# CloudEngineHub/MARL-LLM

Measured on AMD Instinct MI355X. Metric: agent-steps/sec, higher is better.
Workload: dtype f64 (state, every index / flag / reward decision) + f32 (obs, prior, action I/O, pre-filters); 1 GPU; assembly env, 64 agents x 4096 envs per GPU (64 x 4096 total), assembled state, prior-policy actions; agents=64, envs_per_gpu=4096, envs_total=4096, obs_dtype=f32, state_dtype=f64, seed=226, parallelism=env-sharded x1, no collective on the step path

## Files before the change

marl_llm_amd/csrc/swarm_env.hip:

```cpp

#include <hip/hip_runtime.h>

#include <cmath>
#include <cstdint>
#include <cstring>
#include <string>
#include <type_traits>
#include <utility>

#include "swarm_env.h"
#include "env_types.h"

using namespace swarm_internal;

#if !defined(SWARM_ENV_UNIT)
#define SWARM_UNIT_KERNELS 1
#define SWARM_UNIT_HOST 1
#elif SWARM_ENV_UNIT == 0
#define SWARM_UNIT_KERNELS 0
#define SWARM_UNIT_HOST 1
#else
#define SWARM_UNIT_KERNELS 1
#define SWARM_UNIT_HOST 0
#endif
// ... 725 lines not shown
                d2u = (act && up != 0) ? fmaf(dxu, dxu, dy2) : INFINITY;
                d2d = (act && dn != 0) ? fmaf(dxd, dxd, dy2) : INFINITY;
                c_dn = rs[b] + popc(dn) - 1;
            };
            for (int b = wr; b < nr_hi; b += WS) {
                float d2d, d2u; int c_dn;
                row_cands(b, d2d, d2u, c_dn);
                second32 = __builtin_amdgcn_fmed3f(best32, second32, d2d);
                bool lt = d2d < best32;
                best32 = lt ? d2d : best32; bc = lt ? c_dn : bc;
                second32 = __builtin_amdgcn_fmed3f(best32, second32, d2u);
                lt = d2u < best32;
                best32 = lt ? d2u : best32; bc = lt ? c_dn + 1 : bc;
            }
            const float lat_dlt = 1.2e-7f * fmaxf(fabsf(apf), fabsf(bpf)) + 2e-6f;
            const float tol = 6.0f * sqrtf(second32) * lat_dlt + 1e-9f;
            const bool unc_min = act && (wave_exact || (second32 < INFINITY && (second32 - best32) <= tol));
            if (__any(unc_min)) {
                if (unc_min) {
                    const float thr = wave_exact ? INFINITY : best32 + tol;
                    double bestd = INFINITY; int bcd = bc;
                    for (int b = wr; b < nr_hi; b += WS) {
                        float d2d, d2u; int c_dn;
                        row_cands(b, d2d, d2u, c_dn);
                        const bool td = d2d <= thr, tu = d2u <= thr && d2u < INFINITY;
                        if ((td && d2d < INFINITY) || tu) {
                            const double2 g0 = cell64((td && d2d < INFINITY) ? c_dn : 0), g1 = cell64(tu ? c_dn + 1 : 0);
                            const double e0x = g0.x - px, e0y = g0.y - py, e1x = g1.x - px, e1y = g1.y - py;
                            const double q0 = e0x * e0x + e0y * e0y, q1 = e1x * e1x + e1y * e1y;
                            if (td && d2d < INFINITY && q0 < bestd) { bestd = q0; bcd = c_dn; }
                            if (tu && q1 < bestd) { bestd = q1; bcd = c_dn + 1; }
                        }
                    }
                    bc = bcd;
                }
            }
        }
        };
        if (sx != SB || WPE == 1) { if (P.lat_n32) walk(0u); else walk((u64)0); }
    } else {
    for (int rep = 0, reps = REPS(3); rep < reps; ++rep) {
    FENCE();
    best32 = INFINITY; second32 = INFINITY; bc = 0;
    for (int w = 0; w < W; ++w) {
        if (!mine(w)) continue;
        unsigned word = 0, rword = 0;
        int mlo = 0, mhi = 0;
        int bl = 0; const float best_in = best32;
        unsigned orw = 0;
        const unsigned nlo = (unsigned)nearby1, nhi = (unsigned)(nearby1 >> 32);
        u64 unc = 0;
        const float4 *cq = reinterpret_cast<const float4 *>(cq_e + w * 64);
        static_for<16>([&](auto prc) {
            constexpr int pr = decltype(prc)::value;
            const float4 q = cq[pr];
            const f2v gx = {q.x, q.y}, gy = {q.z, q.w};
            const f2v rx = gx - pxx, ry = gy - pyy;
            const f2v d2v = __builtin_elementwise_fma(rx, rx, ry * ry);
            static_for<2>([&](auto hc) {
                constexpr int hh = decltype(hc)::value;
                constexpr int b = 2 * pr + hh;
                const float d2 = hh ? d2v.y : d2v.x;
                second32 = __builtin_amdgcn_fmed3f(best32, second32, d2);
                const bool lt = d2 < best32;
                best32 = lt ? d2 : best32;
                bl = lt ? b : bl;
                const u64 m_slo = __ballot(d2 < P.csen_lo), m_shi = __ballot(d2 < P.csen_hi);
                const u64 m_olo = __ballot(d2 < P.cocc_lo), m_ohi = __ballot(d2 < P.cocc_hi);
                rword = shl1_or_mask(rword, m_slo);
                if constexpr (NW == 1) {
                    const unsigned t = ((unsigned)m_olo & nlo) | ((unsigned)(m_olo >> 32) & nhi);
                    orw = shl1_or_mask(orw, __ballot(t != 0));
                } else {
                    mlo = writelane_c<b>((int)(unsigned)m_olo, mlo);
                    mhi = writelane_c<b>((int)(unsigned)(m_olo >> 32), mhi);
                }
                unc |= (m_slo ^ m_shi) | (m_olo ^ m_ohi);
            });
        });
        word = __brev(rword);
        unsigned oword = __brev(orw);
        if (best32 < best_in) bc = w * 32 + bl;
        u64 mym = ((u64)(unsigned)mhi << 32) | (unsigned)mlo;
        if (unc != 0 || wave_exact) {
            word = 0; oword = 0;
#pragma unroll 4
            for (int b = 0; b < 32; ++b) {
                const double2 g = cell64(w * 32 + b);
                const double rx = g.x - px, ry = g.y - py;
                const double d2 = rx * rx + ry * ry;
                if (d2 < P.c_sen) word |= 1u << b;
                const u64 m = __ballot(d2 < P.c_occ);
                if (lane == b) mym = m;
                if (NW == 1 && ((((unsigned)m & nlo) | ((unsigned)(m >> 32) & nhi)) != 0)) oword |= 1u << b;
            }
        }
        sbits[w * AG + at] = word;
        if constexpr (NW == 1) owords[w * AG + at] = oword;
        else if (lane < 32) cmask[(size_t)(w * 32 + lane) * NW + aw] = mym;
    }
    }
    {
        const float tol = P.min_tol_a * sqrtf(second32) + P.min_tol_b * second32 + 1e-9f;
        const bool unc_min = act && (wave_exact || (second32 < INFINITY && (second32 - best32) <= tol));
        if (__any(unc_min)) {
            const float thr = unc_min ? (wave_exact ? INFINITY : best32 + tol) : -1.0f;
            double bestd = INFINITY; int bcd = bc;
            for (int w = 0; w < W; ++w) {
                if (!mine(w)) continue;
                for (int b = 0; b < 32; ++b) {
                    const int cc = w * 32 + b;
                    const float rx = cq_e[(cc >> 1) * 4 + (cc & 1)] - pxf, ry = cq_e[(cc >> 1) * 4 + 2 + (cc & 1)] - pyf;
                    if (fmaf(rx, rx, ry * ry) <= thr || (wave_exact && unc_min)) {
                        const double2 g = cell64(w * 32 + b);
                        const double ex = g.x - px, ey = g.y - py;
                        const double d2 = ex * ex + ey * ey;
                        if (d2 < bestd) { bestd = d2; bcd = w * 32 + b; }
                    }
                }
            }
            if (unc_min) bc = bcd;
        }
    }
    }
    part_c[sx * AG + at] = (pc_t)bc;
    double *part_d = reinterpret_cast<double *>(smem + LO(partd));
    if constexpr (LAT) {
        if (sx != SB || WPE == 1) {
            const double2 g = cell64(bc);
            const double ex = g.x - px, ey = g.y - py;
            part_d[(WPE > 1 && sx > SB ? sx - 1 : sx) * AG + at] = ex * ex + ey * ey;
        }
    }
    STAMP(16);
    EXIT_AT(4);
    __syncthreads();
    STAMP(17);
    double best = INFINITY; bc = 0;
    for (int rep = 0, reps = REPS(12); rep < reps; ++rep) {
    FENCE();
    best = INFINITY; bc = 0;
#pragma unroll
    for (int s = 0; s < WPE; ++s) {
        if (LAT && WPE > 1 && s == SB) continue;
        const int c = part_c[s * AG + at];
        double d;
        if constexpr (LAT) d = part_d[(WPE > 1 && s > SB ? s - 1 : s) * AG + at];
        else { const double2 g = cell64(c); const double ex = g.x - px, ey = g.y - py; d = ex * ex + ey * ey; }
        if (d < best || (d == best && c < bc)) { best = d; bc = c; }
    }
    }
    const bool in_shape = act && best < P.c_in[es];
    if (sx == 0) {
        sncf[at] = bc | (in_shape ? (1 << 30) : 0);
        if (P.export_small && act) {
            P.near_cell[(size_t)e * n_a + i] = bc;
            P.in_flag[(size_t)e * n_a + i] = in_shape ? 1 : 0;
        }
    }
    STAMP(4);
    EXIT_AT(5);

    const int PPR = P.obs_dim >> 1;
    const int HP = 2 * (P.with_self + P.topo) + 2;
    const int envs_here = (P.n_env - blockIdx.x * EPB) < EPB ? (P.n_env - blockIdx.x * EPB) : EPB;
    const int rows = envs_here * n_a;
    OT2 *out = reinterpret_cast<OT2 *>(obs) + (size_t)blockIdx.x * EPB * n_a * PPR;

    auto prior_policy = [&]() {
    if (sx == SB && P.with_prior) {
        double qx = 0.0, qy = 0.0;
        double lx = 0.0, ly = 0.0;
        {
            const int ncf = sncf[at];
            double tx = px - px, ty = py - py;
            if (!(ncf >> 30)) { const double2 g = cell64(ncf & 0xFFFF); tx = g.x - px; ty = g.y - py; }
            const double dt_ = sqrt(tx * tx + ty * ty);
            if (dt_ > 0) { qx += P.pk_att * tx / dt_; qy += P.pk_att * ty / dt_; }
            lx = qx; ly = qy;
            double avx = 0.0, avy = 0.0; int cnt = 0;
#pragma unroll
            for (int k = 0; k < kTopoMax; ++k) {
                const int j = snei[at * kNeiStride + k];
                const bool used = j >= 0;
                const int tj = el * NPAD + (used ? j : 0);
                const double x = px - sp[tj], y = py - sp[AG + tj];
                const double d2n = x * x + y * y;
                if (used && d2n > 0 && d2n < P.c_avoid) {
                    const double d = sqrt(d2n);
                    const double ux = x / d, uy = y / d;
                    const double factor = P.pk_rep * (P.r_avoid / d - 1.0);
                    qx += factor * ux; qy += factor * uy;
                    if (P.llm) { const double fl = P.pk_llm * (P.r_avoid / d - 1.0); lx += fl * ux; ly += fl * uy; }
                }
                if (used) { avx += sp[2 * AG + tj]; avy += sp[3 * AG + tj]; ++cnt; }
            }
            if (cnt > 0) {
                avx /= cnt; avy /= cnt;
                const double sxv = P.pk_ali * (avx - sp[2 * AG + at]), syv = P.pk_ali * (avy - sp[3 * AG + at]);
                qx += sxv; qy += syv; lx += sxv; ly += syv;
            }
        }
        if (act) {
            OT2 o; o.x = to_out<OT>(clamp_ref(qx, -1.0, 1.0)); o.y = to_out<OT>(clamp_ref(qy, -1.0, 1.0));
            reinterpret_cast<OT2 *>(P.prior_next)[(size_t)e * n_a + i] = o;
            if (P.llm) { double2 u; u.x = clamp_ref(lx, -1.0, 1.0); u.y = clamp_ref(ly, -1.0, 1.0); P.act_next[(size_t)e * n_a + i] = u; }
        }
    }
    };

    auto head_blocks = [&](bool early) {
        for (int rep = 0, reps = REPS(7); rep < reps; ++rep) {
            FENCE();
            typedef OT OT4 __attribute__((ext_vector_type(4)));
            const int NB = P.with_self + P.topo + 1;
            const int total = rows * NB;
            const bool b_out = WPE > 1 && P.with_prior != 0;
            const int HT = b_out ? T - AG : T;
            const int ps = tid / AG, ps_b = (SB + WPE - (int)(blockIdx.x % WPE)) % WPE;
            const int htid = b_out ? (ps < ps_b ? ps : ps - 1) * AG + at : tid;
            const int n_it = early ? (total + 63) >> 6 : (total + HT - 1) / HT;
            for (int it_ = 0; it_ < n_it; ++it_) {
                int item;
                if (early) {
                    const int c8 = it_ & 7, owner = c8 < 5 ? 0 : 2;
                    const int k = owner == 0 ? 5 * (it_ >> 3) + c8 : 3 * (it_ >> 3) + c8 - 5;
                    if (sx != owner || (k % NW) != aw) continue;
                    item = it_ * 64 + lane;
                } else {
                    if (b_out && sx == SB) break;
                    item = htid + it_ * HT;
                }
                if (item < total) {
                    const int r = NB == 8 ? item >> 3 : item / NB, blk = item - r * NB;
                    const int elr = EPB > 1 ? r / n_a : 0;
                    const int tr = elr * NPAD + (r - elr * n_a);
                    const double ox = sp[tr], oy = sp[AG + tr], ou = sp[2 * AG + tr], ov = sp[3 * AG + tr];
                    const bool is_tgt = blk == NB - 1, is_nei = !is_tgt && !(P.with_self && blk == 0);
                    const int nslot = blk - P.with_self;
                    const int j = snei[tr * kNeiStride + (is_nei ? nslot : 0)];
                    const int ncf = sncf[tr];
                    const double2 g = P.cells_xy[(size_t)(blockIdx.x * EPB + elr) * P.ng_max + (ncf & 0xFFFF)];
                    const int tj = elr * NPAD + (j < 0 ? 0 : j);
                    const double nx = sp[tj], ny = sp[AG + tj], nu = sp[2 * AG + tj], nv = sp[3 * AG + tj];
                    const bool has = is_nei && j >= 0, out_t = is_tgt && !(ncf >> 30);
                    const bool zero_m = is_nei && !has;
                    double mx = has ? nx : (out_t ? g.x : ox), my = has ? ny : (out_t ? g.y : oy);
                    double mu = has ? nu : (out_t ? 0.0 : ou), mv = has ? nv : (out_t ? 0.0 : ov);
                    if (zero_m) { mx = 0.0; my = 0.0; mu = 0.0; mv = 0.0; }
                    const bool sub_own = has || is_tgt;
                    const double qx = sub_own ? ox : 0.0, qy = sub_own ? oy : 0.0, qu = sub_own ? ou : 0.0, qv = sub_own ? ov : 0.0;
                    double a = mx - qx, b = my - qy;
                    if (P.periodic && is_nei) wrap_rel(a, b, P.w_half, P.h_half);
                    OT2 *dst = out + (size_t)r * PPR + 2 * blk;
                    if ((PPR & 1) == 0) {
                        const OT4 o = {to_out<OT>(a), to_out<OT>(b), to_out<OT>(mu - qu), to_out<OT>(mv - qv)};
                        __builtin_nontemporal_store(o, reinterpret_cast<OT4 *>(dst));
                    } else {
                        OT2 o0, o1;
                        o0.x = to_out<OT>(a); o0.y = to_out<OT>(b); o1.x = to_out<OT>(mu - qu); o1.y = to_out<OT>(mv - qv);
                        store_nt(dst, o0); store_nt(dst + 1, o1);
                    }
                }
            }
        }
    };

    auto exact_uniform = [&](int La, int nL, int eL) -> bool {
        const double inv_dsen = 1.0 / P.d_sen;
        const double2 *gcl = P.cells_xy + (size_t)eL * P.ng_max;
        const double pxl = sp[La], pyl = sp[AG + La];
        const short *rowl = sidx + (size_t)La * P.g_stride;
        auto bcast = [](double v, int t) -> double {
            const u64 b = __builtin_bit_cast(u64, v);
            const unsigned lo = (unsigned)__builtin_amdgcn_readlane((int)(unsigned)b, t);
            const unsigned hi = (unsigned)__builtin_amdgcn_readlane((int)(unsigned)(b >> 32), t);
            return __builtin_bit_cast(double, ((u64)hi << 32) | lo);
        };
        double a0 = 0.0, a1 = 0.0, a2 = 0.0;
        for (int base = 0; base < nL; base += 64) {
            const int q = base + lane;
            double t0 = 0.0, t1 = 0.0, t2 = 0.0;
            if (q < nL) {
                const int cc = rowl[q];
                const double2 gq = gcl[cc];
                const double x = gq.x - pxl, y = gq.y - pyl;
                const double z = sqrt(x * x + y * y);
                const double psi = z < P.d_sen ? 0.5 * (1.0 + cospi01(z * inv_dsen)) : 0.0;
                t0 = psi * x; t1 = psi * y; t2 = psi;
            }
            const int m = nL - base < 64 ? nL - base : 64;
            for (int t = 0; t < m; ++t) { a0 += bcast(t0, t); a1 += bcast(t1, t); a2 += bcast(t2, t); }
        }
        if (a2 == 0) a2 = 1E-8;
        const double v0 = 1.0 * a0 / a2, v1 = 1.0 * a1 / a2;
        return sqrt(v0 * v0 + v1 * v1) < 0.05;
    };

    auto sensed_rows = [&](bool own, const unsigned char *pw) {
        for (int rep = 0, reps = REPS(8); rep < reps; ++rep) {
            FENCE();
            const int Gp = P.g_max;
            const int wv = __builtin_amdgcn_readfirstlane(tid >> 6), nwv = T >> 6;
            auto locate = [&](int k, int &tr, int &elr, int &r) -> bool {
                if (own) {
                    const int ta = (at & ~63) + pw[(64 - ACTW) + sx * AGW + k];
                    const int ii = NPAD < 64 ? (ta & 63) % NPAD : ta;
                    elr = NPAD < 64 ? (ta & 63) / NPAD : 0;
                    tr = ta; r = elr * n_a + ii;
                    return (blockIdx.x * EPB + elr) < P.n_env && ii < n_a;
                }
                r = k;
                const bool ok = r < rows;
                const int rq = ok ? r : rows - 1;
                elr = EPB > 1 ? rq / n_a : 0;
                tr = elr * NPAD + (rq - elr * n_a);
                return ok;
            };
            if (Gp == 80 && sizeof(OT) <= 4) {
                typedef OT OT4 __attribute__((ext_vector_type(4)));
                const int ngrp = own ? AGW / 8 : (rows + nwv * 8 - 1) / (nwv * 8);
                for (int g8 = 0; g8 < ngrp; ++g8) {
#pragma unroll
                    for (int ps = 0; ps < 5; ++ps) {
                        const int ch = ps * 64 + lane;
                        const int rl = (ch * 205) >> 13;
                        const int m = ch - rl * 40;
                        int tr, elr, r;
                        const bool ok = locate(own ? g8 * 8 + rl : (wv + g8 * nwv) * 8 + rl, tr, elr, r);
                        const double2 *gr = P.cells_xy + (size_t)(blockIdx.x * EPB + elr) * P.ng_max;
                        const double qx = sp[tr], qy = sp[AG + tr];
                        const int cc = *reinterpret_cast<const int *>(sidx + (size_t)tr * P.g_stride + 2 * m);
                        const int c0 = (int)(short)(cc & 0xFFFF), c1 = cc >> 16;
                        const double2 g0 = gr[c0 < 0 ? 0 : c0], g1 = gr[c1 < 0 ? 0 : c1];
                        const OT z = to_out<OT>(0.0);
                        const OT a0 = to_out<OT>(g0.x - qx), b0 = to_out<OT>(g0.y - qy);
                        const OT a1 = to_out<OT>(g1.x - qx), b1 = to_out<OT>(g1.y - qy);
                        OT4 o = {c0 >= 0 ? a0 : z, c0 >= 0 ? b0 : z, c1 >= 0 ? a1 : z, c1 >= 0 ? b1 : z};
                        if (ok) __builtin_nontemporal_store(o, reinterpret_cast<OT4 *>(out + (size_t)r * PPR + HP + 2 * m));
                    }
                }
            } else {
                const int nrow = own ? AGW : (rows - wv + nwv - 1) / nwv;
                for (int k = 0; k < nrow; ++k) {
                    int tr, elr, r;
                    const bool ok = locate(own ? k : wv + k * nwv, tr, elr, r);
                    const double2 *gr = P.cells_xy + (size_t)(blockIdx.x * EPB + elr) * P.ng_max;
                    const double qx = sp[tr], qy = sp[AG + tr];
                    const short *srw = sidx + (size_t)tr * P.g_stride;
                    for (int q = lane; q < Gp; q += 64) {
                        const int c = srw[q];
                        const double2 g = gr[c < 0 ? 0 : c];
                        OT2 o; o.x = c >= 0 ? to_out<OT>(g.x - qx) : to_out<OT>(0.0); o.y = c >= 0 ? to_out<OT>(g.y - qy) : to_out<OT>(0.0);
                        if (ok) store_nt(&out[(size_t)r * PPR + HP + q], o);
                    }
                }
            }
        }
    };

    const int G = P.g_max;
    int n_sel = 0;
    bool uniform = false, unsure = false;
    if constexpr (LAT) {
    const float4 hq = hdr[at];
    const int hb0 = __float_as_int(hq.z), hca0 = __float_as_int(hq.w);
    const LatEnv &L = P.lat[es];
    const u64 *rm = lrm + el * 64;
    const short *rs = lrs + el * 64;
    const bool flg = flag_get();
    for (int rep = 0, reps = REPS(4); rep < reps; ++rep) {
        FENCE();
        for (int t = sx; t < P.lat_nrs; t += WPE) {
            const int b = hb0 + t;
            const int bq = b < 0 ? 0 : (b > 63 ? 63 : b);
            const unsigned sel = srow[t * AG + at] & 0x1FFFFu;
            const u64 rowm = rm[bq];
            const int base = rs[bq] + __popcll(rowm & ((1ull << hca0) - 1ull));
            unsigned kept = sel;
            if (in_shape) {
                const unsigned cv = (unsigned)(covrow[el * 64 + bq] >> hca0);
                kept = sel & ~cv;
                if (flg) {
                    const unsigned relm = (unsigned)(rowm >> hca0);
                    unsigned it = sel & cv;
                    kept = sel;
                    while (it) {
                        const int c = __ffs(it) - 1; it &= it - 1;
                        const double2 g = cell64(base + __popc(relm & ((1u << c) - 1u)));
                        bool occ = false;
                        for (int q = 0; q < NW && !occ; ++q) {
                            u64 nbm = NW == 1 ? (nearby1 >> (NPAD < 64 ? el * NPAD : 0)) : snear[q * AG + at];
                            while (nbm && !occ) {
                                const int j = q * 64 + __ffsll((unsigned long long)nbm) - 1; nbm &= nbm - 1;
                                const double ex = g.x - spx[j], ey = g.y - spy[j];
                                occ = ex * ex + ey * ey < P.c_occ;
                            }
                        }
                        if (occ) kept &= ~(1u << c);
                    }
                }
            }
            if (rep == reps - 1) srow[t * AG + at] = kept | ((unsigned)base << 17);
            pcr[at * NRC + t] = (unsigned char)__popc(kept);
            if (P.export_idx) orow[t * AG + at] = sel & ~kept;
        }
    }
    {
        uint4 *fill = reinterpret_cast<uint4 *>(sidx);
        const int n16 = (AG * P.g_stride * 2) >> 4;
        for (int q = tid; q < n16; q += T) fill[q] = uint4{0xFFFFFFFFu, 0xFFFFFFFFu, 0xFFFFFFFFu, 0xFFFFFFFFu};
    }
    __syncthreads();
    STAMP(5);
    EXIT_AT(6);

    pc_t *prk = part_c;
    int n_kept;
    {
        const uint4 cq = reinterpret_cast<const uint4 *>(pcr)[at];
        n_kept = (int)__builtin_amdgcn_sad_u8(cq.x, 0u, __builtin_amdgcn_sad_u8(cq.y, 0u, __builtin_amdgcn_sad_u8(cq.z, 0u, __builtin_amdgcn_sad_u8(cq.w, 0u, 0u))));
        const int key = (lane < ACTW) ? n_kept * 64 + lane : lane - 64;
        int cnt = 0;
#pragma unroll
        for (int q = 0; q < 16; ++q) cnt += (__builtin_amdgcn_readlane(key, sx * 16 + q) < key) ? 1 : 0;
        prk[sx * AG + at] = (pc_t)cnt;
    }
    n_sel = n_kept > G ? G : n_kept;
    __syncthreads();
    STAMP(18);
    EXIT_AT(7);
    int ea;
    {
        int rank = 0;
#pragma unroll
        for (int s = 0; s < WPE; ++s) rank += prk[s * AG + at];
        unsigned char *pw = perm + (tid >> 6) * 64;
        pw[rank] = (unsigned char)lane;
        __builtin_amdgcn_fence(__ATOMIC_RELEASE, "wavefront");
        __builtin_amdgcn_wave_barrier();
        __builtin_amdgcn_fence(__ATOMIC_ACQUIRE, "wavefront");
        ea = (at & ~63) + pw[(64 - ACTW) + sx * AGW + lane / LPA];
    }
    { if (sx == 3) __builtin_amdgcn_s_setprio(3); else if (sx == 2) __builtin_amdgcn_s_setprio(2); else if (sx == SB) __builtin_amdgcn_s_setprio(1); }

    float qn0 = 0.0f, qn1 = 0.0f, qdn = 0.0f, qrl = 1.0f; int qnk = 0;
    for (int rep = 0, reps = REPS(11); rep < reps; ++rep) {
        FENCE();
        const int sub = lane & (LPA - 1);
        const float4 ha = hdr[ea];
        const float apr = ha.x, bpr = ha.y;
        const int ab0 = __float_as_int(ha.z), aca0 = __float_as_int(ha.w);
        const int ael = NPAD < 64 ? (ea & 63) / NPAD : 0;
        const LatEnv &La = P.lat[(blockIdx.x * EPB + ael) < P.n_env ? (blockIdx.x * EPB + ael) : P.n_env - 1];
        const float Rl = La.R;
        const float inv_r = __builtin_amdgcn_rcpf(Rl);
        const float apr_s = apr * inv_r;
        const u64 *rma = lrm + ael * 64;
        const uint4 cq = reinterpret_cast<const uint4 *>(pcr)[ea];
        const int s0 = (int)__builtin_amdgcn_sad_u8(cq.x, 0u, 0u), s1 = (int)__builtin_amdgcn_sad_u8(cq.y, 0u, 0u);
        const int s2 = (int)__builtin_amdgcn_sad_u8(cq.z, 0u, 0u), s3 = (int)__builtin_amdgcn_sad_u8(cq.w, 0u, 0u);
        const int nk = s0 + s1 + s2 + s3;
        const int per = (nk + LPA - 1) / LPA;
        const int k0 = sub * per < nk ? sub * per : nk;
        const int k1 = k0 + per < nk ? k0 + per : nk;
        int t, before;
        {
            const int c1 = s0, c2 = s0 + s1, c3 = c2 + s2;
            const int d = (k0 >= c1 ? 1 : 0) + (k0 >= c2 ? 1 : 0) + (k0 >= c3 ? 1 : 0);
            before = d == 0 ? 0 : (d == 1 ? c1 : (d == 2 ? c2 : c3));
            const unsigned wd = d == 0 ? cq.x : (d == 1 ? cq.y : (d == 2 ? cq.z : cq.w));
            const int e1 = before + (int)(wd & 255u), e2 = e1 + (int)((wd >> 8) & 255u), e3 = e2 + (int)((wd >> 16) & 255u);
            const int j = (k0 >= e1 ? 1 : 0) + (k0 >= e2 ? 1 : 0) + (k0 >= e3 ? 1 : 0);
            before = j == 0 ? before : (j == 1 ? e1 : (j == 2 ? e2 : e3));
            t = 4 * d + j;
        }
        const unsigned *srp = srow + t * AG + ea;
        const unsigned wd0 = *srp;
        unsigned kept = k0 < k1 ? (wd0 & 0x1FFFFu) : 0u;
        {
            int pb = 0, left = k0 - before;
#pragma unroll
            for (int sh = 16; sh >= 1; sh >>= 1) {
                const int c = __popc((kept >> pb) & ((1u << sh) - 1u));
                const bool go = left >= c;
                left -= go ? c : 0; pb += go ? sh : 0;
            }
            kept &= ~((1u << pb) - 1u);
        }
        int base = (int)(wd0 >> 17);
        const int bt0 = ab0 + t;
        const u64 *rmp = rma + (bt0 < 0 ? 0 : (bt0 > 63 ? 63 : bt0));
        unsigned relm = (unsigned)(*rmp >> aca0);
        float dbf = ((float)t - bpr) * inv_r, db2 = dbf * dbf;
        float n0 = 0.0f, n1 = 0.0f, dn = 0.0f;
        short *row = sidx + (size_t)ea * P.g_stride;
        const unsigned nm1 = (unsigned)(nk - 1);
        auto rank_of = [&](int q) -> int {
            if (P.cap_int) {
                const unsigned x = 2u * (unsigned)q * nm1 + (unsigned)(G - 1);
                const unsigned hq_ = __umulhi(x, P.cap_magic);
                return (int)((((x - hq_) >> 1) + hq_) >> P.cap_shift);
            }
            const double v = q * ((double)nm1 / (G - 1));
            return (int)(P.cap_even ? rint(v) : round(v));
        };
        auto walk_range = [&](auto capped) {
            constexpr bool CAP = decltype(capped)::value;
            int k = k0;
            int slot = k0, nxt = 0;
            if constexpr (CAP) {
                if (nk > G) {
                    if (P.cap_int) slot = k0 > 0 ? (int)((unsigned)((2 * k0 - 1) * (G - 1) + 2 * (int)nm1 - 1) / (2u * nm1)) : 0;
                    else { slot = 0; while (slot < G && rank_of(slot) < k0) ++slot; }
                    slot = slot < G ? slot : G;
                    nxt = slot < G ? rank_of(slot) : 0x7FFFFFFF;
                }
            }
            while (__any(k < k1)) {
                if (k < k1) {
                    if (kept == 0) {
                        srp += AG; ++rmp;
                        const unsigned wd = *srp;
                        kept = wd & 0x1FFFFu; base = (int)(wd >> 17);
                        relm = (unsigned)(*rmp >> aca0);
                        dbf += inv_r; db2 = dbf * dbf;
                    }
                    if (kept != 0) {
                        const int c = __ffs(kept) - 1;
                        kept &= kept - 1;
                        const int cell = base + __popc(relm & ((1u << c) - 1u));
                        bool take = true;
                        if constexpr (CAP) {
                            if (nk > G) {
                                take = k == nxt;
                                if (take) nxt = slot + 1 < G ? rank_of(slot + 1) : 0x7FFFFFFF;
                            }
                        }
                        if constexpr (CAP) { if (take) row[slot] = (short)cell; slot += take ? 1 : 0; }
                        else row[k] = (short)cell;
                        ++k;
                        const float da = fmaf((float)c, inv_r, -apr_s);
                        const float u = fmaf(da, da, db2);
                        float psi = psi5_u_f32(u);
                        if constexpr (CAP) psi = take ? psi : 0.0f;
                        n0 = fmaf(psi, da, n0); n1 = fmaf(psi, dbf, n1); dn += psi;
                    }
                }
            }
        };
        if (__any(nk > G)) walk_range(std::true_type{}); else walk_range(std::false_type{});
        auto quad_sum = [](float v) -> float {
            v += __int_as_float(__builtin_amdgcn_update_dpp(0, __float_as_int(v), 0xB1, 0xF, 0xF, true));
            v += __int_as_float(__builtin_amdgcn_update_dpp(0, __float_as_int(v), 0x4E, 0xF, 0xF, true));
            return v;
        };
        auto lanes_sum = [&](float v) -> float {
            v = quad_sum(v);
            if constexpr (LPA == 8) v += __int_as_float(__builtin_amdgcn_update_dpp(0, __float_as_int(v), 0x104, 0xF, 0xF, true));
            return v;
        };
        qn0 = lanes_sum(n0); qn1 = lanes_sum(n1); qdn = lanes_sum(dn); qnk = nk; qrl = Rl;
    }
    STAMP(19);
    EXIT_AT(9);
    __builtin_amdgcn_fence(__ATOMIC_RELEASE, "wavefront");
    __builtin_amdgcn_wave_barrier();
    __builtin_amdgcn_fence(__ATOMIC_ACQUIRE, "wavefront");
    {
        const int nsl = qnk > G ? G : qnk;
        const bool in_a = (sncf[ea] >> 30) != 0;
        const int ael = NPAD < 64 ? (ea & 63) / NPAD : 0, ai = NPAD < 64 ? (ea & 63) % NPAD : ea;
        const int ae = blockIdx.x * EPB + ael;
        const bool lead = (lane & (LPA - 1)) == 0 && ae < P.n_env && ai < n_a;
        const bool has = lead && in_a && nsl > 0;
        const float thr = P.rew_thr_k;
        const float idn = __builtin_amdgcn_rcpf(qdn);
        const float v0f = qn0 * idn, v1f = qn1 * idn;
        const float vf = sqrtf(fmaf(v0f, v0f, v1f * v1f));
        bool uni = has && vf < thr;
        const float inv_rl = __builtin_amdgcn_rcpf(qrl);
        const bool uns = has && (P.force_exact || !(qdn > 1e-6f) || !(fabsf(vf - thr) > (P.rew_ga_lat * (float)nsl * idn + P.rew_gb_lat) * inv_rl * 1.0001f));
        u64 um = __ballot(uns);
        while (um != 0) {
            const int L = __ffsll((unsigned long long)um) - 1;
            um &= um - 1;
            const bool res = exact_uniform(__builtin_amdgcn_readlane(ea, L), __builtin_amdgcn_readlane(nsl, L), __builtin_amdgcn_readlane(ae, L));
            if (lane == L) uni = res;
        }
        if (lead) {
            const size_t oi = (size_t)ae * n_a + ai;
            if (reward != nullptr) __builtin_nontemporal_store((in_a && !(snei[ea * kNeiStride + kTopoMax] != 0) && uni) ? 1.0f : 0.0f, &reward[oi]);
            if (done != nullptr) __builtin_nontemporal_store((uint8_t)0, &done[oi]);
        }
    }
    STAMP(6);
    EXIT_AT(10);
    prior_policy();
    if (obs != nullptr) {
        head_blocks(NW == 1);
        STAMP(9);
        EXIT_AT(11);
        sensed_rows(true, perm + (tid >> 6) * 64);
    }
    } else {
    {
        u64 nearby[NW];
#pragma unroll
        for (int q = 0; q < NW; ++q) nearby[q] = (NW > 1 && in_shape) ? snear[q * AG + at] : 0;
        for (int rep = 0, reps = REPS(4); rep < reps; ++rep)
        for (int w = 0; w < W; ++w) {
            if (!mine(w)) continue;
            FENCE();
            const unsigned word = sbits[w * AG + at];
            unsigned kw = word;
            if constexpr (NW == 1) {
                if (in_shape) kw = word & ~owords[w * AG + at];
                if (rep == reps - 1) sbits[w * AG + at] = kw;
            } else if (in_shape) {
                unsigned it = word;
                while (it) {
                    int bb[4]; bool occ[4];
#pragma unroll
                    for (int u = 0; u < 4; ++u) { bb[u] = it ? __ffs(it) - 1 : -1; it &= it - 1; }
#pragma unroll
                    for (int u = 0; u < 4; ++u) {
                        const int c = w * 32 + (bb[u] < 0 ? 0 : bb[u]);
                        occ[u] = false;
#pragma unroll
                        for (int q = 0; q < NW; ++q) occ[u] = occ[u] || ((cmask[(size_t)c * NW + q] & nearby[q]) != 0);
                    }
#pragma unroll
                    for (int u = 0; u < 4; ++u) if (bb[u] >= 0 && occ[u]) kw &= ~(1u << bb[u]);
                }
                if (rep == reps - 1) sbits[w * AG + at] = kw;
            }
            asm volatile("" :: "v"(kw));
            if (P.export_idx) obits[w * AG + at] = word & ~kw;
            pc[w * AG + at] = (unsigned char)__popc(kw);
        }
    }
    __syncthreads();
    STAMP(5);
    EXIT_AT(6);

    int n_kept = 0;
    for (int w = 0; w < W; ++w) n_kept += pc[w * AG + at];
    n_sel = n_kept > G ? G : n_kept;
    unsigned *rsel = reinterpret_cast<unsigned *>(smem + P.off_cmask);
    for (int w = sx; w <= W; w += WPE) rsel[w * AG + at] = 0;
    __syncthreads();
    const bool any_sub = __any(n_kept > G) != 0;
    int *sub_base = reinterpret_cast<int *>(smem + P.off_partc);
// ... 476 lines not shown
```

Baseline: 3.143 billion agent-steps/s.

## Software-pipeline the sensed-cell row gather with a four-deep load queue

For the own-agent path with full 64-agent padding, the 80-cell sensed-row emission is rewritten as a three-stage software pipeline. Index loads, the gathers of cell coordinates and the subtract/store are each issued DEPTH=4 passes ahead, with byte-offset arithmetic done in 24-bit multiplies and a separate unpredicated variant for fully populated blocks. The aim is to hide global-memory gather latency and cut per-pass address math. In exchange it adds register pressure and inline-asm scheduling constraints that may lower occupancy.

```diff
diff --git a/marl_llm_amd/csrc/swarm_env.hip b/marl_llm_amd/csrc/swarm_env.hip
--- a/marl_llm_amd/csrc/swarm_env.hip
+++ b/marl_llm_amd/csrc/swarm_env.hip
@@ -1051,9 +1051,11 @@
             FENCE();
             const int Gp = P.g_max;
             const int wv = __builtin_amdgcn_readfirstlane(tid >> 6), nwv = T >> 6;
+            constexpr bool PIPE = NPAD == 64 && !HALF;
+            const unsigned char *pws = !own ? pw : (PIPE ? perm + wv * 64 : pw) + (64 - ACTW) + sx * AGW;
             auto locate = [&](int k, int &tr, int &elr, int &r) -> bool {
                 if (own) {
-                    const int ta = (at & ~63) + pw[(64 - ACTW) + sx * AGW + k];
+                    const int ta = (at & ~63) + pws[k];
                     const int ii = NPAD < 64 ? (ta & 63) % NPAD : ta;
                     elr = NPAD < 64 ? (ta & 63) / NPAD : 0;
                     tr = ta; r = elr * n_a + ii;
@@ -1068,36 +1070,122 @@
             };
             if (Gp == 80 && sizeof(OT) <= 4) {
                 typedef OT OT4 __attribute__((ext_vector_type(4)));
-                const int ngrp = own ? AGW / 8 : (rows + nwv * 8 - 1) / (nwv * 8);
-                for (int g8 = 0; g8 < ngrp; ++g8) {
-#pragma unroll
-                    for (int ps = 0; ps < 5; ++ps) {
-                        const int ch = ps * 64 + lane;
-                        const int rl = (ch * 205) >> 13;
-                        const int m = ch - rl * 40;
-                        int tr, elr, r;
-                        const bool ok = locate(own ? g8 * 8 + rl : (wv + g8 * nwv) * 8 + rl, tr, elr, r);
-                        const double2 *gr = P.cells_xy + (size_t)(blockIdx.x * EPB + elr) * P.ng_max;
-                        const double qx = sp[tr], qy = sp[AG + tr];
-                        const int cc = *reinterpret_cast<const int *>(sidx + (size_t)tr * P.g_stride + 2 * m);
-                        const int c0 = (int)(short)(cc & 0xFFFF), c1 = cc >> 16;
-                        const double2 g0 = gr[c0 < 0 ? 0 : c0], g1 = gr[c1 < 0 ? 0 : c1];
-                        const OT z = to_out<OT>(0.0);
-                        const OT a0 = to_out<OT>(g0.x - qx), b0 = to_out<OT>(g0.y - qy);
-                        const OT a1 = to_out<OT>(g1.x - qx), b1 = to_out<OT>(g1.y - qy);
-                        OT4 o = {c0 >= 0 ? a0 : z, c0 >= 0 ? b0 : z, c1 >= 0 ? a1 : z, c1 >= 0 ? b1 : z};
-                        if (ok) __builtin_nontemporal_store(o, reinterpret_cast<OT4 *>(out + (size_t)r * PPR + HP + 2 * m));
+                if (!own || !PIPE) {
+                    const int ngrp = own ? AGW / 8 : (rows + nwv * 8 - 1) / (nwv * 8);
+                    for (int g8 = 0; g8 < ngrp; ++g8) {
+#pragma unroll
+                        for (int ps = 0; ps < 5; ++ps) {
+                            const int ch = ps * 64 + lane;
+                            const int rl = (ch * 205) >> 13;
+                            const int m = ch - rl * 40;
+                            int tr, elr, r;
+                            const bool ok = locate(own ? g8 * 8 + rl : (wv + g8 * nwv) * 8 + rl, tr, elr, r);
+                            const double2 *gr = P.cells_xy + (size_t)(blockIdx.x * EPB + elr) * P.ng_max;
+                            const double qx = sp[tr], qy = sp[AG + tr];
+                            const int cc = *reinterpret_cast<const int *>(sidx + (size_t)tr * P.g_stride + 2 * m);
+                            const int c0 = (int)(short)(cc & 0xFFFF), c1 = cc >> 16;
+                            const double2 g0 = gr[c0 < 0 ? 0 : c0], g1 = gr[c1 < 0 ? 0 : c1];
+                            const OT z = to_out<OT>(0.0);
+                            const OT a0 = to_out<OT>(g0.x - qx), b0 = to_out<OT>(g0.y - qy);
+                            const OT a1 = to_out<OT>(g1.x - qx), b1 = to_out<OT>(g1.y - qy);
+                            OT4 o = {c0 >= 0 ? a0 : z, c0 >= 0 ? b0 : z, c1 >= 0 ? a1 : z, c1 >= 0 ? b1 : z};
+                            if (ok) __builtin_nontemporal_store(o, reinterpret_cast<OT4 *>(out + (size_t)r * PPR + HP + 2 * m));
+                        }
                     }
+                } else {
+                constexpr int ngrp = AGW / 8, NPASS = 5 * ngrp, DEPTH = 4;
+                constexpr int S = (int)sizeof(OT2);
+                const char *gbase = reinterpret_cast<const char *>(P.cells_xy + (size_t)(blockIdx.x * EPB) * P.ng_max);
+                const int e_last = (P.n_env - 1) - (int)(blockIdx.x * EPB);
+                const int a64 = __builtin_amdgcn_readfirstlane(at & ~63);
+                const unsigned row_b = PPR * S, head_b = HP * S, list_b = P.g_stride * 2;
+                int rl = 0, m = 0;
+                auto stage1 = [&](bool pred, int t, int &qo, int &so, int &cc, unsigned &eo) {
+                    if (t % ngrp == 0) {
+                        int ln = lane;
+                        asm volatile("" : "+v"(ln));
+                        const int ch = (t / ngrp) * 64 + ln;
+                        rl = (int)(__umul24(ch, 205) >> 13);
+                        m = ch - rl * 40;
+                    }
+                    const int ta = a64 + pws[(t % ngrp) * 8 + rl];
+                    int elr = NPAD < 64 ? ta / NPAD : 0, r = ta;
+                    bool ok = true;
+                    if (pred) {
+                        const int ii = NPAD < 64 ? ta % NPAD : ta;
+                        r = elr * n_a + ii;
+                        ok = elr <= e_last && ii < n_a;
+                    }
+                    cc = *reinterpret_cast<const int *>(reinterpret_cast<const char *>(sidx) + (__umul24(ta, list_b) + m * 4));
+                    if (pred) {
+                        asm volatile("" : "+v"(cc));
+                        if (!ok) cc = -1;
+                        if (EPB > 1 && elr > e_last) elr = e_last;
+                    }
+                    eo = EPB > 1 ? (unsigned)elr * (unsigned)P.ng_max : 0u;
+                    qo = ta * 8;
+                    so = (int)(__umul24(r, row_b) + (head_b + m * (2 * S)));
+                    if (pred && ok) so |= (int)0x80000000;
+                    asm volatile("" : "+v"(qo), "+v"(so));
+                };
+                auto stage2 = [&](int cc, unsigned eo, double2 &g0, double2 &g1) {
+                    const int c0 = (int)(short)(cc & 0xFFFF), c1 = cc >> 16;
+                    g0 = *reinterpret_cast<const double2 *>(gbase + ((eo + (unsigned)(c0 < 0 ? 0 : c0)) << 4));
+                    g1 = *reinterpret_cast<const double2 *>(gbase + ((eo + (unsigned)(c1 < 0 ? 0 : c1)) << 4));
+                };
+                auto stage3 = [&](int qo, int cc, double2 g0, double2 g1, OT4 &o) {
+                    const int c0 = (int)(short)(cc & 0xFFFF), c1 = cc >> 16;
+                    const char *q = reinterpret_cast<const char *>(sp) + qo;
+                    const double qx = *reinterpret_cast<const double *>(q), qy = *reinterpret_cast<const double *>(q + AG * 8);
+                    const OT z = to_out<OT>(0.0);
+                    const OT a0 = to_out<OT>(g0.x - qx), b0 = to_out<OT>(g0.y - qy);
+                    const OT a1 = to_out<OT>(g1.x - qx), b1 = to_out<OT>(g1.y - qy);
+                    o = OT4{c0 >= 0 ? a0 : z, c0 >= 0 ? b0 : z, c1 >= 0 ? a1 : z, c1 >= 0 ? b1 : z};
+                };
+                typedef std::integral_constant<bool, true> pred_yes;
+                typedef std::integral_constant<bool, false> pred_no;
+                auto groups = [&](auto PRED) {
+                    constexpr bool pred = decltype(PRED)::value;
+                    int qo[DEPTH], so[DEPTH], cc[DEPTH];
+                    double2 ga[DEPTH], gb[DEPTH];
+                    {
+                        unsigned eo[DEPTH];
+#pragma unroll
+                        for (int t = 0; t < DEPTH; ++t) stage1(pred, t, qo[t], so[t], cc[t], eo[t]);
+#pragma unroll
+                        for (int t = 0; t < DEPTH; ++t) stage2(cc[t], eo[t], ga[t], gb[t]);
+                    }
+                    __builtin_amdgcn_sched_barrier(0);
+#pragma unroll
+                    for (int t = 0; t < NPASS; ++t) {
+                        const int k = t % DEPTH;
+                        const bool more = t + DEPTH < NPASS;
+                        int qn = 0, sn = 0, cn = 0;
+                        unsigned en = 0;
+                        if (more) stage1(pred, t + DEPTH, qn, sn, cn, en);
+                        if constexpr (pred) asm volatile("" : "+v"(ga[k].x), "+v"(ga[k].y), "+v"(gb[k].x), "+v"(gb[k].y));
+                        OT4 o;
+                        stage3(qo[k], cc[k], ga[k], gb[k], o);
+                        const int sk = so[k];
+                        if (more) { qo[k] = qn; so[k] = sn; cc[k] = cn; stage2(cn, en, ga[k], gb[k]); }
+                        OT4 *dst = reinterpret_cast<OT4 *>(reinterpret_cast<char *>(out) + (unsigned)(pred ? sk & 0x7FFFFFFF : sk));
+                        if (!pred || sk < 0) __builtin_nontemporal_store(o, dst);
+                    }
+                };
+                if (n_a == NPAD && (int)(blockIdx.x * EPB) + EPB <= P.n_env) groups(pred_no{});
+                else groups(pred_yes{});
                 }
             } else {
                 const int nrow = own ? AGW : (rows - wv + nwv - 1) / nwv;
+                int l0 = lane;
+                if constexpr (PIPE) asm volatile("" : "+v"(l0));
                 for (int k = 0; k < nrow; ++k) {
                     int tr, elr, r;
                     const bool ok = locate(own ? k : wv + k * nwv, tr, elr, r);
                     const double2 *gr = P.cells_xy + (size_t)(blockIdx.x * EPB + elr) * P.ng_max;
                     const double qx = sp[tr], qy = sp[AG + tr];
                     const short *srw = sidx + (size_t)tr * P.g_stride;
-                    for (int q = lane; q < Gp; q += 64) {
+                    for (int q = l0; q < Gp; q += 64) {
                         const int c = srw[q];
                         const double2 g = gr[c < 0 ? 0 : c];
                         OT2 o; o.x = c >= 0 ? to_out<OT>(g.x - qx) : to_out<OT>(0.0); o.y = c >= 0 ? to_out<OT>(g.y - qy) : to_out<OT>(0.0);
```

Result: faster. 3.255 billion agent-steps/s (median of 6 runs) (+3.6%).
